# dharunm236/TempME

Measured on AMD Instinct MI355X. Metric: explained target-edges/sec (TGN+Enron, n_degree=20) at 1/2/4/8 MI355X, higher is better.
Workload: dtype fp32

## Files before the change

tempme_amd/csrc/encoder.hip:

```cpp
#include <algorithm>
#include <atomic>
#include <cstring>
#include <vector>

#include "encoder_common.h"

namespace tmk {

__device__ __forceinline__ double block_sum(double v, double *red) {
#pragma unroll
    for (int o = 32; o > 0; o >>= 1) v += __shfl_xor(v, o);
    const int wave = threadIdx.x >> 6, nw = blockDim.x >> 6;
    __syncthreads();
    if ((threadIdx.x & 63) == 0) red[wave] = v;
    __syncthreads();
    double s = 0.0;
    for (int k = 0; k < nw; ++k) s += red[k];
    return s;
}

__global__ void __launch_bounds__(1024) std_kernel(int32_t B, int32_t W, const double *__restrict__ cut,
                                                   const float *__restrict__ ts3, float *__restrict__ std_out) {
    __shared__ double red[16];
    const int64_t g = blockIdx.x;
// ... 525 lines not shown

template <int NQE>
struct WalkLay {
    static constexpr int EV = FoldLay::SIZE, EVB = EV + 11 * NQE * 256, G1 = EVB + 176, G1B = G1 + 4 * 11 * 256,
                         G2 = G1B + 64, G2B = G2 + 4 * 4 * 256, W1 = G2B + 64, W1B = W1 + 8 * 8 * 256, W2 = W1B + 128,
                         W2B = W2 + 8 * 8 * 256, A1 = W2B + 128, A1B = A1 + 4 * 8 * 256, A2 = A1B + 64,
                         A2B = A2 + 4 * 4 * 256, M1 = A2B + 64, M1B = M1 + 5 * 5 * 256, M2 = M1B + 80,
                         M2B = M2 + 4 * 5 * 256;
};

constexpr int PFP = 4;
constexpr int WALK_WAVES = 2;
constexpr int WALK_WPB = 4;

constexpr int GCN_LDS = 3;
constexpr int GCN_LDS_FRAGS = GCN_LDS * 12;
constexpr int PAIR_LIN_RING = 6, PAIR_GCN_RING = 6;
constexpr int gcn_step(int k, int gl, int ns) {
    const int nstr = ns - gl, m = nstr < gl ? nstr : gl;
    if (k < 2 * m) return (k & 1) ? k / 2 : gl + k / 2;
    return nstr > gl ? gl + k - m : k - m;
}

template <int NTO, int NQ, int NQL, int BASE>
__device__ __forceinline__ void cgemm(__amdgpu_buffer_rsrc_t wr, const floatx4 (&x)[NQ], floatx4 (&o)[NTO]) {
    using O = PairOrder<NTO, NQ>;
    const int vo = lane_id() * 16;
    constexpr int N = NTO * NQ, D = PFP < N ? PFP : N;
    auto off = [](int i) { return BASE / 4 + (O::t(i) * NQL + O::q(i)) * 64; };
    float4 buf[D];
#pragma unroll
// ... 283 lines not shown
    const float4 v = erow4[i < n4 ? i : n4 - 1];
    return i < n4 ? v : make_float4(0.f, 0.f, 0.f, 0.f);
}

#define ETAB_N(q0) ((q0) > 0 ? 11 : 1)
template <int Q0>
__device__ __forceinline__ void load_et(const WalkArgs &a, int32_t e, float4 (&et)[ETAB_N(Q0)]) {
    if constexpr (Q0 > 0) {
        const float4 *trow = reinterpret_cast<const float4 *>(a.etab + (int64_t)e * 176);
        const int g = lane_id() >> 4;
#pragma unroll
        for (int t = 0; t < 11; ++t) et[t] = trow[4 * t + g];
    }
}

template <int NTD, bool AGAIN, int D, class Extra>
__device__ __forceinline__ void gcn_zn(__amdgpu_buffer_rsrc_t wr, int vog, const float4 *gl, const floatx4 (&L)[NTD],
                                       float4 (&gb)[D], Extra &&extra, floatx4 (&Hs)[4], float4 (&pre)[PFP],
                                       const NextFr &nx) {
    constexpr int NSG = (NTD + 1) / 2, GL = GCN_LDS, N = (NSG - GL) * 12;
    static_assert(N % D == 0 && D >= PFP, "event_gcn ring depth");
    const int vo = lane_id() * 16, ln = lane_id();
    auto goff = [](int i) { return ((((i / 3) % 4) * NSG + GL + i / 12) * 3 + i % 3) * 64; };
    int zg = 0;
    asm volatile("" : "+s"(zg));
    auto wloadg = [&](int i) {
        return __builtin_bit_cast(float4, __builtin_amdgcn_raw_buffer_load_b128(wr, vog, zg + goff(i) * 16, 0));
    };
    auto take = [&](int i) {
        const float4 v = gb[i % D];
        if (i + D < N) gb[i % D] = wloadg(i + D);
        else if constexpr (AGAIN) gb[i % D] = wloadg(i + D - N);
        else if (i + D - N < PFP) gb[i % D] = wload(wr, vo, nx.o[i + D - N]);
        return v;
    };
    auto fetch = [&](int p, float4 (&w)[6]) {
        const int u = gcn_step(p / 2, GL, NSG), t = 2 * (p & 1);
#pragma unroll
        for (int k = 0; k < 6; ++k) {
            if (u < GL) w[k] = gl[((u * 4 + t) * 3 + k) * 64 + ln];
            else w[k] = take(((u - GL) * 4 + t) * 3 + k);
        }
    };
    auto act = [&](Split3 &x, int u, int j) {
        const int q = 2 * u + (j >> 2);
        if (q < NTD) {
            split_put(x, j, 0.f + relu(0.f + L[q < NTD ? q : 0][j & 3]));
        } else {
            x.h[j] = (__bf16)0.f;
            x.m[j] = (__bf16)0.f;
            x.l[j] = (__bf16)0.f;
        }
    };
    Split3 xb;
#pragma unroll
    for (int j = 0; j < 8; ++j) act(xb, gcn_step(0, GL, NSG), j);
    float4 wb[2][6];
    fetch(0, wb[0]);
#pragma unroll
    for (int k = 0; k < NSG; ++k) {
        extra(2 * k);
        if (2 * k + 1 < NTD) extra(2 * k + 1);
        Split3 xn = xb;
#pragma unroll
        for (int t = 0; t < 4; t += 2) {
            const int pp = 2 * k + t / 2;
            if (pp + 1 < 2 * NSG) fetch(pp + 1, wb[(pp + 1) & 1]);
            const float4(&w)[6] = wb[pp & 1];
            const bf16x8 h0 = __builtin_bit_cast(bf16x8, w[0]), m0 = __builtin_bit_cast(bf16x8, w[1]),
                         l0 = __builtin_bit_cast(bf16x8, w[2]), h1 = __builtin_bit_cast(bf16x8, w[3]),
                         m1 = __builtin_bit_cast(bf16x8, w[4]), l1 = __builtin_bit_cast(bf16x8, w[5]);
            Hs[t] = TM_MF32(l0, xb.h, Hs[t]);
            Hs[t + 1] = TM_MF32(l1, xb.h, Hs[t + 1]);
            Hs[t] = TM_MF32(h0, xb.l, Hs[t]);
            Hs[t + 1] = TM_MF32(h1, xb.l, Hs[t + 1]);
            Hs[t] = TM_MF32(m0, xb.m, Hs[t]);
            Hs[t + 1] = TM_MF32(m1, xb.m, Hs[t + 1]);
            Hs[t] = TM_MF32(m0, xb.h, Hs[t]);
            Hs[t + 1] = TM_MF32(m1, xb.h, Hs[t + 1]);
            Hs[t] = TM_MF32(h0, xb.m, Hs[t]);
            Hs[t + 1] = TM_MF32(h1, xb.m, Hs[t + 1]);
            Hs[t] = TM_MF32(h0, xb.h, Hs[t]);
            Hs[t + 1] = TM_MF32(h1, xb.h, Hs[t + 1]);
            if (k + 1 < NSG) {
#pragma unroll
                for (int j = 2 * t; j < 2 * t + 4; ++j) act(xn, gcn_step(k + 1, GL, NSG), j);
            }
            __builtin_amdgcn_sched_barrier(0);
        }
        xb = xn;
    }
    if constexpr (!AGAIN) {
#pragma unroll
        for (int k = 0; k < PFP; ++k) pre[k] = gb[(N + k) % D];
    }
}

template <int NQE, int NTD, bool SEF, int Q0, bool ZN, class Extra>
__device__ __forceinline__ void encode_position(const WalkArgs &a, __amdgpu_buffer_rsrc_t wr, const float *cs,
                                                const PosIn &pi, const float (&ef)[EQ_MAX][4],
                                                float4 (&et)[ETAB_N(Q0)], Extra &&extra, int p, floatx4 (&H)[8],
                                                float4 (&pre)[PFP], const NextFr &nx, unsigned long long (&T)[10],
                                                const float4 *gl) {
    constexpr bool ETAB = Q0 > 0;
    static_assert(!(ETAB && SEF), "table mode replaces the streamed edge features");
    using C = WalkConsts<NQE, NTD>;
    using LY = WalkLay<NQE>;
    const EncW &P = a.P;
    const int g = lane_id() >> 4;
    const int de = P.de, dn = P.dn;
    const float dt = pi.v ? pi.tb - pi.ta : 0.f, c0 = pi.v ? pi.c0 : 0.f, c1 = pi.v ? pi.c1 : 0.f,
                c2 = pi.v ? pi.c2 : 0.f;
    const float4 *nrow_s = reinterpret_cast<const float4 *>(a.n_feat + (int64_t)(pi.v ? pi.ns : 0) * dn);
    const float4 *nrow_t = reinterpret_cast<const float4 *>(a.n_feat + (int64_t)(pi.v ? pi.nt : 0) * dn);
    floatx4 L[NTD];
    if constexpr (ETAB) {
#pragma unroll
        for (int t = 0; t < NTD; ++t) L[t] = floatx4{et[t].x, et[t].y, et[t].z, et[t].w};
        if (p == 2) {
#pragma unroll
            for (int t = 0; t < NTD; ++t) L[t] = add4(L[t], lds4(cs + C::DEVC, t));
        }
    } else {
        const float *bias = cs + (p == 2 ? C::EVC : C::EV);
#pragma unroll
        for (int t = 0; t < NTD; ++t) L[t] = ldsx4(bias, t);
    }
    TM_STAMP(1);
    constexpr int NSG = (NTD + 1) / 2, GD = 12, GL = GCN_LDS;
    static_assert(GL >= 1 && GL < NSG, "event_gcn's resident steps");
    const int vog = lane_id() * 16 + 16 * (int)(P.g13 - P.kv.w);
    auto goff = [](int i) { return ((((i / 3) % 4) * NSG + GL + i / 12) * 3 + i % 3) * 64; };
    float4 gb[ZN ? GD : 1];
    (void)vog, (void)goff, (void)gb;
    constexpr int JN = 3;
    float4 rs[JN], rt[JN];
    auto nload = [&](int q) {
        const int f4 = (q < NTD - 1) ? 4 * q + g : min(4 * q + g, dn / 4 - 1);
        rs[q % JN] = nrow_s[f4];
        rt[q % JN] = nrow_t[f4];
    };
    {
        constexpr int NS = C::NS, S0 = Q0 / 2;
        constexpr int N = NTD * (NS - S0) * 3, D = 12;
        static_assert(D >= PFP && D <= N && D % 3 == 0, "lin_event ring depth");
        static_assert(D == GD, "the zero-node event_gcn takes over lin_event's ring slots");
        const int vo = lane_id() * 16;
        const int vo3 = vo + 16 * (int)(P.ev3 - P.kv.w);
// ... 47 lines not shown
                        e2[1] = ef_step(erow4, s + 2, 1, g, de);
                    }
                }
                Split3 xn = xs;
                auto gen = [&](int j) {
                    if (s + 1 < NS && j < 8) {
                        const float e = edge(s + 1, j);
                        const float v = pure(s + 1) ? gen_one<ETAB, true>(s + 1, j, w8[j], p8[j], e, g, de, dt, c0, c1, c2)
                                                    : gen_one<ETAB, false>(s + 1, j, w8[j], p8[j], e, g, de, dt, c0, c1, c2);
                        split_put(xn, j, v);
                    }
                };
                auto take = [&](int i) {
                    const bf16x8 v = __builtin_bit_cast(bf16x8, buf[i % D]);
                    if (i + D < N) buf[i % D] = wload3(i + D);
                    else if constexpr (ZN) buf[i % D] = wloadg(i + D - N);
                    else if (i + D - N < PFP) buf[i % D] = wload(wr, vo, g1f(i + D - N));
                    return v;
                };
#pragma unroll
                for (int t = 0; t + 1 < NTD; t += 2) {
                    const int i = ((s - S0) * NTD + t) * 3;
                    const bf16x8 h0 = take(i), m0 = take(i + 1), l0 = take(i + 2);
                    const bf16x8 h1 = take(i + 3), m1 = take(i + 4), l1 = take(i + 5);
                    L[t] = TM_MF32(l0, xs.h, L[t]);
                    L[t + 1] = TM_MF32(l1, xs.h, L[t + 1]);
                    L[t] = TM_MF32(h0, xs.l, L[t]);
                    L[t + 1] = TM_MF32(h1, xs.l, L[t + 1]);
                    L[t] = TM_MF32(m0, xs.m, L[t]);
                    L[t + 1] = TM_MF32(m1, xs.m, L[t + 1]);
                    L[t] = TM_MF32(m0, xs.h, L[t]);
// ... 14 lines not shown
                    L[t] = TM_MF32(h0, xs.l, L[t]);
                    L[t] = TM_MF32(m0, xs.m, L[t]);
                    L[t] = TM_MF32(m0, xs.h, L[t]);
                    L[t] = TM_MF32(h0, xs.m, L[t]);
                    L[t] = TM_MF32(h0, xs.h, L[t]);
                    gen(t);
                    __builtin_amdgcn_sched_barrier(0);
                }
                if constexpr (SEF) {
                    ring[s & 1][0] = e2[0];
                    ring[s & 1][1] = e2[1];
                }
                xs = xn;
            }
        }
        if constexpr (ZN) {
            if (p == 2) {
#pragma unroll
                for (int k = 0; k < D; ++k) buf[(N + k) % D] = wloadg(k);
            }
#pragma unroll
            for (int k = 0; k < D; ++k) gb[k] = buf[(N + k) % D];
        } else {
            if (p == 2) {
#pragma unroll
                for (int k = 0; k < PFP; ++k) buf[(N + k) % D] = wload(wr, vo, g1f(k));
            }
#pragma unroll
            for (int k = 0; k < PFP; ++k) pre[k] = buf[(N + k) % D];
        }
    }
    TM_STAMP(2);
    floatx4 Hs[4], Ht[4];
#pragma unroll
    for (int t = 0; t < 4; ++t) {
        Hs[t] = ldsx4(cs + C::G1, t);
        if constexpr (!ZN) Ht[t] = ldsx4(cs + C::G1C, t);
    }
    if constexpr (ZN) {
        gcn_zn<NTD, false, GD>(wr, vog, gl, L, gb, extra, Hs, pre, nx);
    } else {
        const int vo = lane_id() * 16;
        float4 wq[2][4];
        {
#pragma unroll
            for (int q = 0; q < JN - 1 && q < NTD; ++q) nload(q);
        }
#pragma unroll
        for (int t = 0; t < 4; ++t) wq[0][t] = pre[t];
#pragma unroll
        for (int q = 0; q < NTD; ++q) {
            if (q + JN - 1 < NTD) nload(q + JN - 1);
            if (q + 1 < NTD) {
#pragma unroll
                for (int t = 0; t < 4; ++t) wq[(q + 1) & 1][t] = wload(wr, vo, LY::G1 / 4 + (t * NTD + q + 1) * 64);
// ... 26 lines not shown
            __builtin_amdgcn_sched_barrier(0);
        }
#pragma unroll
        for (int t = 0; t < 4; ++t) pre[t] = wq[NTD & 1][t];
    }
    TM_STAMP(3);
    TM_STAMP(4);
#pragma unroll
    for (int t = 0; t < 4; ++t) {
        H[t] = relu4(Hs[t]);
        H[4 + t] = ZN ? H[t] : relu4(Ht[t]);
    }
    TM_STAMP(5);
}

template <int NQE, int NTD, int Q0, class Extra>
__device__ __forceinline__ void encode_pair(const WalkArgs &a, __amdgpu_buffer_rsrc_t wr, const float *cs,
                                            const PosIn &pi0, const PosIn &pi1, const float4 (&et0)[NTD],
                                            const float4 (&et1)[NTD], Extra &&extra, floatx4 (&U0)[4],
                                            floatx4 (&U1)[4], float4 (&pre)[PFP], const NextFr &nx,
                                            unsigned long long (&T)[10], const float4 *gl) {
    static_assert(Q0 > 0, "the pair pass starts from the edge table's rows");
    using C = WalkConsts<NQE, NTD>;
    const EncW &P = a.P;
    const int g = lane_id() >> 4;
    const int de = P.de;
    const float dt0 = pi0.v ? pi0.tb - pi0.ta : 0.f, c00 = pi0.v ? pi0.c0 : 0.f, c01 = pi0.v ? pi0.c1 : 0.f,
                c02 = pi0.v ? pi0.c2 : 0.f;
    const float dt1 = pi1.v ? pi1.tb - pi1.ta : 0.f, c10 = pi1.v ? pi1.c0 : 0.f, c11 = pi1.v ? pi1.c1 : 0.f,
                c12 = pi1.v ? pi1.c2 : 0.f;
    floatx4 L0[NTD], L1[NTD];
#pragma unroll
    for (int t = 0; t < NTD; ++t) {
        L0[t] = floatx4{et0[t].x, et0[t].y, et0[t].z, et0[t].w};
        L1[t] = floatx4{et1[t].x, et1[t].y, et1[t].z, et1[t].w};
    }
    TM_STAMP(1);
    constexpr int NSG = (NTD + 1) / 2, GL = GCN_LDS;
    const int vog = lane_id() * 16 + 16 * (int)(P.g13 - P.kv.w);
    constexpr int GD = PAIR_GCN_RING;
    float4 gb[GD];
    {
        constexpr int NS = C::NS, S0 = Q0 / 2;
        constexpr int N = NTD * (NS - S0) * 3, D = PAIR_LIN_RING;
        static_assert(D >= PFP && D <= N && D % 3 == 0 && D <= GD, "lin_event ring depth");
        const int vo3 = lane_id() * 16 + 16 * (int)(P.ev3 - P.kv.w);
        auto off = [](int i) { return ((((i / 3) % NTD) * NS + S0 + i / (3 * NTD)) * 3 + i % 3) * 64; };
        auto goff = [](int i) { return ((((i / 3) % 4) * NSG + GL + i / 12) * 3 + i % 3) * 64; };
        int z3 = 0;
        asm volatile("" : "+s"(z3));
        auto wload3 = [&](int i) {
            return __builtin_bit_cast(float4, __builtin_amdgcn_raw_buffer_load_b128(wr, vo3, z3 + off(i) * 16, 0));
        };
        auto wloadg = [&](int i) {
            return __builtin_bit_cast(float4, __builtin_amdgcn_raw_buffer_load_b128(wr, vog, z3 + goff(i) * 16, 0));
        };
        float4 buf[D];
#pragma unroll
        for (int i = 0; i < D; ++i) buf[i] = i < PFP ? pre[i] : wload3(i);
        auto pure = [](int s) { return s > S0; };
        const float *cw = cs + C::XW, *cp = cs + C::XP;
        Split3 xs0, xs1;
        {
            float w8[8], p8[8];
            lds8(cw, S0, w8);
            lds8(cp, S0, p8);
#pragma unroll
            for (int j = 0; j < 8; ++j) {
                split_put(xs0, j, gen_one<true, false>(S0, j, w8[j], p8[j], 0.f, g, de, dt0, c00, c01, c02));
                split_put(xs1, j, gen_one<true, false>(S0, j, w8[j], p8[j], 0.f, g, de, dt1, c10, c11, c12));
            }
// ... 3 lines not shown
            Split3 xn0 = xs0, xn1 = xs1;
            auto gen = [&](int j) {
                if (s + 1 < NS && j < 8) {
                    const float w = cw[32 * (s + 1) + 8 * g + j], ph = cp[32 * (s + 1) + 8 * g + j];
                    const float v0 = pure(s + 1) ? gen_one<true, true>(s + 1, j, w, ph, 0.f, g, de, dt0, c00, c01, c02)
                                                 : gen_one<true, false>(s + 1, j, w, ph, 0.f, g, de, dt0, c00, c01, c02);
                    const float v1 = pure(s + 1) ? gen_one<true, true>(s + 1, j, w, ph, 0.f, g, de, dt1, c10, c11, c12)
                                                 : gen_one<true, false>(s + 1, j, w, ph, 0.f, g, de, dt1, c10, c11, c12);
                    split_put(xn0, j, v0);
                    split_put(xn1, j, v1);
                }
            };
            auto take = [&](int i) {
                const bf16x8 v = __builtin_bit_cast(bf16x8, buf[i % D]);
                if (i + D < N) buf[i % D] = wload3(i + D);
                else buf[i % D] = wloadg(i + D - N);
                return v;
            };
#pragma unroll
            for (int t = 0; t < NTD; ++t) {
                const int i = ((s - S0) * NTD + t) * 3;
                const bf16x8 h = take(i), m = take(i + 1), l = take(i + 2);
                L0[t] = TM_MF32(l, xs0.h, L0[t]);
                L1[t] = TM_MF32(l, xs1.h, L1[t]);
                L0[t] = TM_MF32(h, xs0.l, L0[t]);
                L1[t] = TM_MF32(h, xs1.l, L1[t]);
                L0[t] = TM_MF32(m, xs0.m, L0[t]);
                L1[t] = TM_MF32(m, xs1.m, L1[t]);
                L0[t] = TM_MF32(m, xs0.h, L0[t]);
                L1[t] = TM_MF32(m, xs1.h, L1[t]);
                L0[t] = TM_MF32(h, xs0.m, L0[t]);
                L1[t] = TM_MF32(h, xs1.m, L1[t]);
                L0[t] = TM_MF32(h, xs0.h, L0[t]);
                L1[t] = TM_MF32(h, xs1.h, L1[t]);
                gen(t);
                __builtin_amdgcn_sched_barrier(0);
            }
            xs0 = xn0;
            xs1 = xn1;
        }
#pragma unroll
        for (int k = 0; k < GD; ++k) gb[k] = k < D ? buf[(N + k) % D] : wloadg(k);
    }
    TM_STAMP(2);
    floatx4 Hs[4];
#pragma unroll
    for (int t = 0; t < 4; ++t) Hs[t] = ldsx4(cs + C::G1, t);
    gcn_zn<NTD, true, GD>(wr, vog, gl, L0, gb, [](int) {}, Hs, pre, nx);
#pragma unroll
    for (int t = 0; t < 4; ++t) U0[t] = relu4(Hs[t]);
    TM_STAMP(3);
#pragma unroll
    for (int t = 0; t < 4; ++t) Hs[t] = ldsx4(cs + C::G1, t);
    gcn_zn<NTD, false, GD>(wr, vog, gl, L1, gb, extra, Hs, pre, nx);
    TM_STAMP(4);
#pragma unroll
    for (int t = 0; t < 4; ++t) U1[t] = relu4(Hs[t]);
    TM_STAMP(5);
}

__device__ __forceinline__ float col_sum(float v) {
    v += __shfl_xor(v, 16);
    v += __shfl_xor(v, 32);
    return v;
}

struct HeadIn {
    double cu;
    float sd, t0, t1;
// ... 105 lines not shown
__device__ __forceinline__ float score_dot(const Stash<ZN ? 4 : 8> &st, const floatx4 (&H)[NH]) {
    static_assert(NH >= (ZN ? 4 : 8), "a position's hidden vector");
    const int lane = threadIdx.x & 63;
    float s = 0.f;
#pragma unroll
    for (int t = 0; t < (ZN ? 4 : 8); ++t) {
        const floatx4 v = st.V[t][lane];
#pragma unroll
        for (int r = 0; r < 4; ++r) s = __builtin_fmaf(v[r], H[t][r], s);
    }
    return col_sum(s) + st.cw[lane];
}

template <int NQE, int NTD, bool SEF = false, int QE0 = 0, bool SPLIT = false, bool ZN = false, bool POOL = false,
          bool PAIR = false>
__global__ void __launch_bounds__(64 * WALK_WPB, 4 * WALK_WAVES / WALK_WPB) walk_kernel(WalkArgs a) {
    static_assert(!PAIR || (ZN && QE0 > 0 && !SEF && !POOL), "the pair pass: zero-node table mode, not pooled");
    using C = WalkConsts<NQE, NTD>;
    constexpr int NA = ZN ? 4 : 8;
    const EncW &P = a.P;
    const int lane = threadIdx.x & 63, col = lane & 15;
    const int32_t NS = a.W / a.M;
    const int64_t n_units = (a.n_slots + 15) / 16;
    constexpr bool PERSIST = !SPLIT;
    const int64_t ustride = PERSIST ? (int64_t)gridDim.x * (blockDim.x >> 6) : n_units;
    int64_t unit = (int64_t)blockIdx.x * (blockDim.x >> 6) + (threadIdx.x >> 6);
    auto ticket = [&]() -> int64_t {
        uint32_t t = 0;
        if (lane == 0) t = atomicAdd(a.ticket, 1u);
        return ustride + (int64_t)(uint32_t)__builtin_amdgcn_readfirstlane((int)t);
    };
    int m0 = 0;
    if constexpr (SPLIT) {
        m0 = (int)(unit % a.M);
        unit /= a.M;
    }
    auto coords = [&](int64_t u, bool &v, int64_t &eg_, int32_t &j_) {
        const int64_t gs = u * 16 + col;
        v = u < n_units && gs < a.n_slots;
        eg_ = v ? gs / NS : 0;
        j_ = v ? (int32_t)(gs % NS) : 0;
    };
    bool valid;
    int64_t eg;
    int32_t j;
    coords(unit, valid, eg, j);
    __shared__ Stash<NA> stash[WALK_WPB];
    __shared__ float4 cs4[(C::SIZE + 3) / 4];
    float *cs = reinterpret_cast<float *>(cs4);
#ifdef TM_TRACE
    const int64_t trw = (int64_t)blockIdx.x * (blockDim.x >> 6) + (threadIdx.x >> 6);
    int trn = 0;
    const unsigned long long tr0 = __builtin_amdgcn_s_memrealtime();
#endif
    __shared__ float4 gl[ZN ? GCN_LDS_FRAGS * 64 : 1];
    if constexpr (ZN) {
        constexpr int NSG = (NTD + 1) / 2;
        for (int i = threadIdx.x; i < GCN_LDS_FRAGS * 64; i += blockDim.x) {
            const int f = i >> 6, l = i & 63;
            gl[i] = P.g13[((((f / 3) % 4) * NSG + f / 12) * 3 + f % 3) * 64 + l];
        }
    }
    load_consts<NQE, NTD, ZN>(P, cs);
    __syncthreads();
#ifdef TM_TRACE
    if (lane == 0 && trw < 8192) {
        g_tr[trw][0] = tr0;
        g_tr[trw][1] = __builtin_amdgcn_s_memrealtime();
        g_tr[trw][28] = 0;
        g_tr[trw][29] = (unsigned)__builtin_amdgcn_s_getreg(63492) | ((unsigned long long)(unsigned)__builtin_amdgcn_s_getreg(30740) << 32);
    }
#endif
    if (unit >= n_units) return;
// ... 61 lines not shown
        const int64_t gwn = !last ? eg * a.W + (int64_t)j * a.M + (SPLIT ? m0 : PAIR ? pass : pass >> 1)
                                  : egn * a.W + (int64_t)jn * a.M;
        PosIn nxt, nxt1;
        auto extra = [&](int q) {
            if (q == 0) {
                load_hi();
                nxt = load_pos(a, gwn, pn, !last ? valid : vn);
                if constexpr (PAIR) nxt1 = load_pos(a, gwn, 1, !last ? valid : vn);
            }
        };
        unsigned long long T[10];
        TM_STAMP(0);
        if (PAIR && pt == 3) {
            if constexpr (PAIR) {
                floatx4 U0[4], U1[4];
                encode_pair<NQE, NTD, QE0>(a, wr, cs, cur, cur1, et, et1, extra, U0, U1, pre,
                                           pair_first<4>(FoldLay::A1GZ / 4), T, gl);
                load_et<QE0>(a, nxt.edge(), et);
                load_et<QE0>(a, nxt1.edge(), et1);
                cur = nxt;
                cur1 = nxt1;
                TM_STAMP(6);
                const float sc0 = score_dot<true>(st, U0), sc1 = score_dot<true>(st, U1);
                TM_STAMP(7);
                walk_head<NQE, NTD, true>(a, wr, cs, gw, valid, hi, st, sc0, sc1, U0, U1, pre, lin0);
            }
        } else {
        const int p = PAIR ? 2 : pt;
        floatx4 H[8];
        const NextFr nx_pos = ZN ? pair_first<4>(p == 2 ? FoldLay::A1DZ / 4 : FoldLay::A1GZ / 4)
                                 : pair_first<8>(p == 2 ? FoldLay::A1D / 4 : FoldLay::A1G / 4);
        encode_position<NQE, NTD, SEF, QE0, ZN>(a, wr, cs, cur, ef, et, extra, p, H, pre,
                                                p == 0 ? lin0 : nx_pos, T, gl);
        if constexpr (QE0 == 0) load_ef(a, nxt.edge(), ef);
        else load_et<QE0>(a, nxt.edge(), et);
        cur = nxt;
        if constexpr (PAIR) {
            load_et<QE0>(a, nxt1.edge(), et1);
            cur1 = nxt1;
        }
        TM_STAMP(6);
        floatx4 Uv[4];
#pragma unroll
        for (int t = 0; t < 4; ++t) Uv[t] = H[t];
        if (ZN && p == 2) {
            floatx4 P2[4], V[4];
#pragma unroll
// ... 663 lines not shown
                        const uint8_t *drop, float dscale, hipStream_t s) {
    const int tr = head_tr(P);
    if (tr == 32)
        head_kernel<32><<<dim3((unsigned)((n_walks + 31) / 32)), 256, head_lds(P, 32), s>>>(
            P, n_walks, walks_per_group, W, F, ts3, cut, cat, stdv, out, drop, dscale);
    else
        head_kernel<16><<<dim3((unsigned)((n_walks + 15) / 16)), 256, head_lds(P, 16), s>>>(
            P, n_walks, walks_per_group, W, F, ts3, cut, cat, stdv, out, drop, dscale);
}

constexpr int64_t WALK_SPLIT_UNITS = 512;

static bool walk_split(int64_t units, int32_t M) { return units * M <= 3 * WALK_SPLIT_UNITS && units < WALK_SPLIT_UNITS; }

template <int NQE, bool SEF, int Q0, bool ZN, bool POOL, bool PAIR>
static void launch_walk_as(const WalkArgs &a, unsigned blocks, hipStream_t s) {
    const int64_t units = (a.n_slots + 15) / 16;
    if (walk_split(units, a.M)) {
        const unsigned sb = (unsigned)((units * a.M + WALK_WPB - 1) / WALK_WPB);
        walk_kernel<NQE, 11, SEF, Q0, true, ZN, POOL, PAIR><<<dim3(sb), 64 * WALK_WPB, 0, s>>>(a);
        return;
    }
    static int cap[64] = {};
    int dev = 0;
    if (hipGetDevice(&dev) == hipSuccess && dev >= 0 && dev < 64) {
        if (cap[dev] == 0) {
            int per_cu = 0, cus = 0;
            if (hipOccupancyMaxActiveBlocksPerMultiprocessor(&per_cu, walk_kernel<NQE, 11, SEF, Q0, false, ZN, POOL, PAIR>, 64 * WALK_WPB, 0) ==
                    hipSuccess &&
                hipDeviceGetAttribute(&cus, hipDeviceAttributeMultiprocessorCount, dev) == hipSuccess && per_cu > 0 &&
                cus > 0)
                cap[dev] = per_cu * cus;
            else
                cap[dev] = -1;
        }
        if (cap[dev] > 0 && blocks > (unsigned)cap[dev]) blocks = (unsigned)cap[dev];
    }
    const int dbg = debug_opt(TM_DEBUG_WALK_BLOCKS);
    if (dbg > 0 && blocks > (unsigned)dbg) blocks = (unsigned)dbg;
    walk_kernel<NQE, 11, SEF, Q0, false, ZN, POOL, PAIR><<<dim3(blocks), 64 * WALK_WPB, 0, s>>>(a);
}

template <int NQE, bool SEF = false, int Q0 = 0, bool ZN = false, bool POOL = false>
static void launch_walk(const WalkArgs &a, unsigned blocks, hipStream_t s) {
    if constexpr (ZN && Q0 > 0 && !SEF && !POOL) {
        if (!debug_opt(TM_DEBUG_WALK_SINGLE)) return launch_walk_as<NQE, SEF, Q0, ZN, POOL, true>(a, blocks, s);
    }
    launch_walk_as<NQE, SEF, Q0, ZN, POOL, false>(a, blocks, s);
}

extern "C" int tm_encoder_fwd(const tm_weights *w, const float *n_feat, const float *e_feat, int32_t n_groups,
                              int32_t B, int32_t W, int32_t M, const int32_t *node6, const int32_t *eid3,
                              const float *ts3, const int32_t *cat, const double *cut, const float *cnt,
                              void *workspace, float *out_imp, void *stream) {
    return tm_encoder_fwd_tab(w, n_feat, e_feat, nullptr, n_groups, B, W, M, node6, eid3, ts3, cat, cut, cnt,
                              workspace, out_imp, stream);
}

static int encoder_fwd_impl(const tm_weights *w, const float *n_feat, const float *e_feat, const float *etab,
                            int32_t n_groups, int32_t B, int32_t W, int32_t M, const int32_t *node6, const int32_t *eid3,
                            const float *ts3, const int32_t *cat, const double *cut, const float *cnt, void *workspace,
                            float *out_imp, void *stream, bool do_std);

// ... 26 lines not shown
        pe = prof_begin(s);
        if (P.tg) std_kernel<<<dim3(n_groups), 1024, 0, s>>>(B, W, cut, ts3, stdv);
        TM_CHECK_LAUNCH();
        prof_end("std_kernel", s, pe);
    }
    if (etab && etab_q0(P) == 0) return fail(TM_E_UNSUPPORTED, "tm_encoder_fwd_tab: no edge table for these dims");
    const int nqe = r16(P.kev) / 16, ntd = r16(P.dn) / 16;
    const bool narrow = nqe >= 11 && nqe <= 14 && P.de <= 16 * EQ_MAX;
    const bool wide = (nqe == 21 || nqe == 22) && P.de > 16 * EQ_MAX && P.de % 4 == 0;
    if (ntd == 11 && P.dn % 4 == 0 && (narrow || wide) && P.h == HID && P.cat) {
        if (!walk_layout_ok(P, nqe)) return fail(TM_E_UNSUPPORTED, "tm_encoder_fwd: weight layout mismatch");
        const int64_t n_slots = n_walks / M;
        const int64_t units = (n_slots + 15) / 16;
        WalkArgs a{P, n_slots, W, M, B * W, n_feat, e_feat, node6, eid3, cat, ts3, cnt, stdv, cut, out_imp, etab,
                   reinterpret_cast<uint32_t *>(F)};
        const unsigned blocks = (unsigned)((units + WALK_WPB - 1) / WALK_WPB);
        const int q0 = etab ? etab_q0(P) : 0;
        if (!walk_split(units, M)) TM_HIP(hipMemsetAsync(a.ticket, 0, sizeof(uint32_t), s));
        pe = prof_begin(s);
        if (q0 == 2 && w->node_zero) {
            if (nqe == 11) launch_walk<11, false, 2, true>(a, blocks, s);
            else if (nqe == 12) launch_walk<12, false, 2, true>(a, blocks, s);
            else if (nqe == 13) launch_walk<13, false, 2, true>(a, blocks, s);
            else launch_walk<14, false, 2, true>(a, blocks, s);
        } else if (q0 == 2) {
            if (nqe == 11) launch_walk<11, false, 2>(a, blocks, s);
            else if (nqe == 12) launch_walk<12, false, 2>(a, blocks, s);
            else if (nqe == 13) launch_walk<13, false, 2>(a, blocks, s);
            else launch_walk<14, false, 2>(a, blocks, s);
        } else if (q0 == 10) {
            if (nqe == 21) launch_walk<21, false, 10>(a, blocks, s);
            else launch_walk<22, false, 10>(a, blocks, s);
        } else if (wide) {
            if (nqe == 21) launch_walk<21, true>(a, blocks, s);
            else launch_walk<22, true>(a, blocks, s);
        } else if (nqe == 11) launch_walk<11>(a, blocks, s);
        else if (nqe == 12) launch_walk<12>(a, blocks, s);
        else if (nqe == 13) launch_walk<13>(a, blocks, s);
        else launch_walk<14>(a, blocks, s);
        TM_CHECK_LAUNCH();
        prof_end("walk_kernel", s, pe);
        return TM_OK;
    }
    const int64_t n_rows = n_walks * 3;
    pe = prof_begin(s);
    launch_gcn(P, w->node_zero, n_rows, lds_g, n_feat, e_feat, node6, eid3, ts3, cnt, F, s);
    TM_CHECK_LAUNCH();
    prof_end("gcn_kernel", s, pe);
    pe = prof_begin(s);
    launch_head(P, n_walks, (int64_t)B * W, W, F, ts3, cut, cat, stdv, out_imp, nullptr, 1.f, s);
    TM_CHECK_LAUNCH();
    prof_end("head_kernel", s, pe);
    return TM_OK;
}

static int64_t pool_part_offset(const tm_weights *w, int64_t n_walks) {
    return (tm_encoder_workspace_bytes(w, n_walks) + 255) & ~(int64_t)255;
}

extern "C" int64_t tm_encoder_pool_workspace_bytes(const tm_weights *w, int64_t n_walks) {
    return pool_part_offset(w, n_walks) + n_walks * (w ? w->h : HID) * (int64_t)sizeof(float) + 256;
}

static void launch_walk_pool(const WalkArgs &a, int nqe, bool wide, int q0, int node_zero, unsigned blocks,
                             hipStream_t s) {
    if (q0 == 2 && node_zero) {
        if (nqe == 11) launch_walk<11, false, 2, true, true>(a, blocks, s);
        else if (nqe == 12) launch_walk<12, false, 2, true, true>(a, blocks, s);
        else if (nqe == 13) launch_walk<13, false, 2, true, true>(a, blocks, s);
        else launch_walk<14, false, 2, true, true>(a, blocks, s);
    } else if (q0 == 2) {
        if (nqe == 11) launch_walk<11, false, 2, false, true>(a, blocks, s);
        else if (nqe == 12) launch_walk<12, false, 2, false, true>(a, blocks, s);
        else if (nqe == 13) launch_walk<13, false, 2, false, true>(a, blocks, s);
        else launch_walk<14, false, 2, false, true>(a, blocks, s);
    } else if (q0 == 10) {
        if (nqe == 21) launch_walk<21, false, 10, false, true>(a, blocks, s);
        else launch_walk<22, false, 10, false, true>(a, blocks, s);
    } else if (wide) {
        if (nqe == 21) launch_walk<21, true, 0, false, true>(a, blocks, s);
        else launch_walk<22, true, 0, false, true>(a, blocks, s);
    } else if (nqe == 11) launch_walk<11, false, 0, false, true>(a, blocks, s);
    else if (nqe == 12) launch_walk<12, false, 0, false, true>(a, blocks, s);
    else if (nqe == 13) launch_walk<13, false, 0, false, true>(a, blocks, s);
    else launch_walk<14, false, 0, false, true>(a, blocks, s);
}

extern "C" int tm_encoder_pool_fwd(const tm_weights *w, const float *n_feat, const float *e_feat, const float *etab,
                                   int32_t n_groups, int32_t B, int32_t W, int32_t M, const int32_t *node6,
                                   const int32_t *eid3, const float *ts3, const int32_t *cat, const double *cut,
                                   const float *cnt, const float *wgt, void *workspace, float *out, int64_t ld_out,
                                   void *stream) {
    if (!w || n_groups < 0 || B < 0 || W < 0 || M <= 0) return fail(TM_E_ARG, "tm_encoder_pool_fwd: bad arguments");
    if (W % M) return fail(TM_E_SHAPE, "tm_encoder_pool_fwd: W must be a multiple of M (walks per hop-1 slot)");
    const int64_t n_walks = (int64_t)n_groups * B * W, n_events = (int64_t)n_groups * B;
    if (n_events == 0) return TM_OK;
    const EncW &P = w->P;
    if (ld_out < P.hm) return fail(TM_E_ARG, "tm_encoder_pool_fwd: ld_out below the row width (hid_dim (+ 12))");
    if (!n_feat || !e_feat || !node6 || !eid3 || !ts3 || !cat || !cut || !cnt || !wgt || !workspace || !out)
        return fail(TM_E_ARG, "tm_encoder_pool_fwd: NULL pointer");
// ... 7 lines not shown
    if (n_walks > 0) {
        hipEvent_t pe = prof_begin(s);
        if (P.tg) std_kernel<<<dim3(n_groups), 1024, 0, s>>>(B, W, cut, ts3, stdv);
        TM_CHECK_LAUNCH();
        prof_end("std_kernel", s, pe);
        if (etab && etab_q0(P) == 0) return fail(TM_E_UNSUPPORTED, "tm_encoder_pool_fwd: no edge table for these dims");
        const int nqe = r16(P.kev) / 16, ntd = r16(P.dn) / 16;
        const bool narrow = nqe >= 11 && nqe <= 14 && P.de <= 16 * EQ_MAX;
        const bool wide = (nqe == 21 || nqe == 22) && P.de > 16 * EQ_MAX && P.de % 4 == 0;
        if (ntd == 11 && P.dn % 4 == 0 && (narrow || wide) && P.h == HID && P.cat) {
            if (!walk_layout_ok(P, nqe)) return fail(TM_E_UNSUPPORTED, "tm_encoder_pool_fwd: weight layout mismatch");
            const int64_t n_slots = n_walks / M;
            const int64_t units = (n_slots + 15) / 16;
            WalkArgs a{P, n_slots, W, M, B * W, n_feat, e_feat, node6, eid3, cat, ts3, cnt, stdv, cut, part, etab,
                       reinterpret_cast<uint32_t *>(F), wgt};
            const unsigned blocks = (unsigned)((units + WALK_WPB - 1) / WALK_WPB);
            const bool split = walk_split(units, M);
            if (!split) TM_HIP(hipMemsetAsync(a.ticket, 0, sizeof(uint32_t), s));
            n_part = split ? W : W / M;
            pe = prof_begin(s);
            launch_walk_pool(a, nqe, wide, etab ? etab_q0(P) : 0, w->node_zero, blocks, s);
            TM_CHECK_LAUNCH();
            prof_end("walk_pool_kernel", s, pe);
        } else {
            pe = prof_begin(s);
            launch_gcn(P, w->node_zero, n_walks * 3, lds_g, n_feat, e_feat, node6, eid3, ts3, cnt, F, s);
            TM_CHECK_LAUNCH();
            prof_end("gcn_kernel", s, pe);
            pe = prof_begin(s);
            head_kernel<16, true><<<dim3((unsigned)((n_walks + 15) / 16)), 256, head_lds(P, 16), s>>>(
                P, n_walks, (int64_t)B * W, W, F, ts3, cut, cat, stdv, part, nullptr, 1.f, wgt);
            TM_CHECK_LAUNCH();
            prof_end("head_pool_kernel", s, pe);
        }
    }
    hipEvent_t pe = prof_begin(s);
// ... 493 lines not shown
```

Before: 3.725 million.

## Keep all GCN weight steps resident in LDS with 8-wave workgroups

For zero-node, non-split walk kernels (pair or pooled), the workgroup grows from 4 to 8 waves and the whole GCN weight tile for all steps is staged in LDS, so gcn_zn no longer streams weight fragments through a register ring from global memory. The ring buffers and their prefetch logic are compiled out in resident mode, and the next-stage prefetch is issued directly instead. This aims to cut repeated global weight loads and free ring registers, at the cost of more LDS per block and changed launch bounds, which may lower occupancy. Launchers now compute the block count from the per-variant waves-per-block.

After: 3.955 million, median of 6. 1.06x the previous value.

```diff
diff --git a/tempme_amd/csrc/encoder.hip b/tempme_amd/csrc/encoder.hip
--- a/tempme_amd/csrc/encoder.hip
+++ b/tempme_amd/csrc/encoder.hip
@@ -563,7 +563,14 @@
 constexpr int WALK_WPB = 4;
 
 constexpr int GCN_LDS = 3;
-constexpr int GCN_LDS_FRAGS = GCN_LDS * 12;
+#ifndef TM_WALK_WG8
+#define TM_WALK_WG8 1
+#endif
+constexpr bool walk_wg8(bool zn, bool pair, bool split, bool pool) { return TM_WALK_WG8 && zn && !split && (pair || pool); }
+constexpr int walk_wpb(bool zn, bool pair, bool split, bool pool) { return walk_wg8(zn, pair, split, pool) ? 8 : WALK_WPB; }
+constexpr int walk_gl(bool zn, bool pair, bool split, bool pool, int nsg) {
+    return walk_wg8(zn, pair, split, pool) ? nsg : GCN_LDS;
+}
 constexpr int PAIR_LIN_RING = 6, PAIR_GCN_RING = 6;
 constexpr int gcn_step(int k, int gl, int ns) {
     const int nstr = ns - gl, m = nstr < gl ? nstr : gl;
@@ -877,12 +884,14 @@
     }
 }
 
-template <int NTD, bool AGAIN, int D, class Extra>
+template <int NTD, bool AGAIN, int GL, int D, class Extra>
 __device__ __forceinline__ void gcn_zn(__amdgpu_buffer_rsrc_t wr, int vog, const float4 *gl, const floatx4 (&L)[NTD],
                                        float4 (&gb)[D], Extra &&extra, floatx4 (&Hs)[4], float4 (&pre)[PFP],
                                        const NextFr &nx) {
-    constexpr int NSG = (NTD + 1) / 2, GL = GCN_LDS, N = (NSG - GL) * 12;
-    static_assert(N % D == 0 && D >= PFP, "event_gcn ring depth");
+    constexpr int NSG = (NTD + 1) / 2, N = (NSG - GL) * 12;
+    constexpr bool RES = GL == NSG;
+    static_assert(GL >= 1 && GL <= NSG, "event_gcn's resident steps");
+    static_assert(RES || (N % D == 0 && D >= PFP), "event_gcn ring depth");
     const int vo = lane_id() * 16, ln = lane_id();
     auto goff = [](int i) { return ((((i / 3) % 4) * NSG + GL + i / 12) * 3 + i % 3) * 64; };
     int zg = 0;
@@ -898,10 +907,10 @@
         return v;
     };
     auto fetch = [&](int p, float4 (&w)[6]) {
-        const int u = gcn_step(p / 2, GL, NSG), t = 2 * (p & 1);
+        const int u = gcn_step(p / 2, GCN_LDS, NSG), t = 2 * (p & 1);
 #pragma unroll
         for (int k = 0; k < 6; ++k) {
-            if (u < GL) w[k] = gl[((u * 4 + t) * 3 + k) * 64 + ln];
+            if (RES || u < GL) w[k] = gl[((u * 4 + t) * 3 + k) * 64 + ln];
             else w[k] = take(((u - GL) * 4 + t) * 3 + k);
         }
     };
@@ -917,7 +926,7 @@
     };
     Split3 xb;
 #pragma unroll
-    for (int j = 0; j < 8; ++j) act(xb, gcn_step(0, GL, NSG), j);
+    for (int j = 0; j < 8; ++j) act(xb, gcn_step(0, GCN_LDS, NSG), j);
     float4 wb[2][6];
     fetch(0, wb[0]);
 #pragma unroll
@@ -947,19 +956,19 @@
             Hs[t + 1] = TM_MF32(h1, xb.h, Hs[t + 1]);
             if (k + 1 < NSG) {
 #pragma unroll
-                for (int j = 2 * t; j < 2 * t + 4; ++j) act(xn, gcn_step(k + 1, GL, NSG), j);
+                for (int j = 2 * t; j < 2 * t + 4; ++j) act(xn, gcn_step(k + 1, GCN_LDS, NSG), j);
             }
             __builtin_amdgcn_sched_barrier(0);
         }
         xb = xn;
     }
-    if constexpr (!AGAIN) {
+    if constexpr (!AGAIN && !RES) {
 #pragma unroll
         for (int k = 0; k < PFP; ++k) pre[k] = gb[(N + k) % D];
     }
 }
 
-template <int NQE, int NTD, bool SEF, int Q0, bool ZN, class Extra>
+template <int NQE, int NTD, bool SEF, int Q0, bool ZN, int GL, class Extra>
 __device__ __forceinline__ void encode_position(const WalkArgs &a, __amdgpu_buffer_rsrc_t wr, const float *cs,
                                                 const PosIn &pi, const float (&ef)[EQ_MAX][4],
                                                 float4 (&et)[ETAB_N(Q0)], Extra &&extra, int p, floatx4 (&H)[8],
@@ -990,11 +999,12 @@
         for (int t = 0; t < NTD; ++t) L[t] = ldsx4(bias, t);
     }
     TM_STAMP(1);
-    constexpr int NSG = (NTD + 1) / 2, GD = 12, GL = GCN_LDS;
-    static_assert(GL >= 1 && GL < NSG, "event_gcn's resident steps");
+    constexpr int NSG = (NTD + 1) / 2, GD = 12;
+    constexpr bool RES = ZN && GL == NSG;
+    static_assert(!ZN || (GL >= 1 && GL <= NSG), "event_gcn's resident steps");
     const int vog = lane_id() * 16 + 16 * (int)(P.g13 - P.kv.w);
     auto goff = [](int i) { return ((((i / 3) % 4) * NSG + GL + i / 12) * 3 + i % 3) * 64; };
-    float4 gb[ZN ? GD : 1];
+    float4 gb[ZN && !RES ? GD : 1];
     (void)vog, (void)goff, (void)gb;
     constexpr int JN = 3;
     float4 rs[JN], rt[JN];
@@ -1072,7 +1082,9 @@
                 auto take = [&](int i) {
                     const bf16x8 v = __builtin_bit_cast(bf16x8, buf[i % D]);
                     if (i + D < N) buf[i % D] = wload3(i + D);
-                    else if constexpr (ZN) buf[i % D] = wloadg(i + D - N);
+                    else if constexpr (RES) {
+                        if (i + D - N < PFP) buf[i % D] = wload(wr, vo, nx.o[i + D - N]);
+                    } else if constexpr (ZN) buf[i % D] = wloadg(i + D - N);
                     else if (i + D - N < PFP) buf[i % D] = wload(wr, vo, g1f(i + D - N));
                     return v;
                 };
@@ -1117,7 +1129,14 @@
                 xs = xn;
             }
         }
-        if constexpr (ZN) {
+        if constexpr (RES) {
+            if (p == 2) {
+#pragma unroll
+                for (int k = 0; k < PFP; ++k) buf[(N + k) % D] = wload(wr, vo, nx.o[k]);
+            }
+#pragma unroll
+            for (int k = 0; k < PFP; ++k) pre[k] = buf[(N + k) % D];
+        } else if constexpr (ZN) {
             if (p == 2) {
 #pragma unroll
                 for (int k = 0; k < D; ++k) buf[(N + k) % D] = wloadg(k);
@@ -1141,7 +1160,7 @@
         if constexpr (!ZN) Ht[t] = ldsx4(cs + C::G1C, t);
     }
     if constexpr (ZN) {
-        gcn_zn<NTD, false, GD>(wr, vog, gl, L, gb, extra, Hs, pre, nx);
+        gcn_zn<NTD, false, GL, RES ? 1 : GD>(wr, vog, gl, L, gb, extra, Hs, pre, nx);
     } else {
         const int vo = lane_id() * 16;
         float4 wq[2][4];
@@ -1198,7 +1217,7 @@
     TM_STAMP(5);
 }
 
-template <int NQE, int NTD, int Q0, class Extra>
+template <int NQE, int NTD, int Q0, int GL, class Extra>
 __device__ __forceinline__ void encode_pair(const WalkArgs &a, __amdgpu_buffer_rsrc_t wr, const float *cs,
                                             const PosIn &pi0, const PosIn &pi1, const float4 (&et0)[NTD],
                                             const float4 (&et1)[NTD], Extra &&extra, floatx4 (&U0)[4],
@@ -1220,14 +1239,17 @@
         L1[t] = floatx4{et1[t].x, et1[t].y, et1[t].z, et1[t].w};
     }
     TM_STAMP(1);
-    constexpr int NSG = (NTD + 1) / 2, GL = GCN_LDS;
+    constexpr int NSG = (NTD + 1) / 2;
+    constexpr bool RES = GL == NSG;
     const int vog = lane_id() * 16 + 16 * (int)(P.g13 - P.kv.w);
-    constexpr int GD = PAIR_GCN_RING;
+    constexpr int GD = RES ? 1 : PAIR_GCN_RING;
     float4 gb[GD];
+    (void)vog, (void)gb;
     {
         constexpr int NS = C::NS, S0 = Q0 / 2;
         constexpr int N = NTD * (NS - S0) * 3, D = PAIR_LIN_RING;
-        static_assert(D >= PFP && D <= N && D % 3 == 0 && D <= GD, "lin_event ring depth");
+        static_assert(D >= PFP && D <= N && D % 3 == 0 && (RES || D <= GD), "lin_event ring depth");
+        const int vo = lane_id() * 16;
         const int vo3 = lane_id() * 16 + 16 * (int)(P.ev3 - P.kv.w);
         auto off = [](int i) { return ((((i / 3) % NTD) * NS + S0 + i / (3 * NTD)) * 3 + i % 3) * 64; };
         auto goff = [](int i) { return ((((i / 3) % 4) * NSG + GL + i / 12) * 3 + i % 3) * 64; };
@@ -1239,6 +1261,7 @@
         auto wloadg = [&](int i) {
             return __builtin_bit_cast(float4, __builtin_amdgcn_raw_buffer_load_b128(wr, vog, z3 + goff(i) * 16, 0));
         };
+        (void)wloadg, (void)vo;
         float4 buf[D];
 #pragma unroll
         for (int i = 0; i < D; ++i) buf[i] = i < PFP ? pre[i] : wload3(i);
@@ -1272,7 +1295,9 @@
             auto take = [&](int i) {
                 const bf16x8 v = __builtin_bit_cast(bf16x8, buf[i % D]);
                 if (i + D < N) buf[i % D] = wload3(i + D);
-                else buf[i % D] = wloadg(i + D - N);
+                else if constexpr (RES) {
+                    if (i + D - N < PFP) buf[i % D] = wload(wr, vo, nx.o[i + D - N]);
+                } else buf[i % D] = wloadg(i + D - N);
                 return v;
             };
 #pragma unroll
@@ -1297,20 +1322,25 @@
             xs0 = xn0;
             xs1 = xn1;
         }
-#pragma unroll
-        for (int k = 0; k < GD; ++k) gb[k] = k < D ? buf[(N + k) % D] : wloadg(k);
+        if constexpr (RES) {
+#pragma unroll
+            for (int k = 0; k < PFP; ++k) pre[k] = buf[(N + k) % D];
+        } else {
+#pragma unroll
+            for (int k = 0; k < GD; ++k) gb[k] = k < D ? buf[(N + k) % D] : wloadg(k);
+        }
     }
     TM_STAMP(2);
     floatx4 Hs[4];
 #pragma unroll
     for (int t = 0; t < 4; ++t) Hs[t] = ldsx4(cs + C::G1, t);
-    gcn_zn<NTD, true, GD>(wr, vog, gl, L0, gb, [](int) {}, Hs, pre, nx);
+    gcn_zn<NTD, true, GL, GD>(wr, vog, gl, L0, gb, [](int) {}, Hs, pre, nx);
 #pragma unroll
     for (int t = 0; t < 4; ++t) U0[t] = relu4(Hs[t]);
     TM_STAMP(3);
 #pragma unroll
     for (int t = 0; t < 4; ++t) Hs[t] = ldsx4(cs + C::G1, t);
-    gcn_zn<NTD, false, GD>(wr, vog, gl, L1, gb, extra, Hs, pre, nx);
+    gcn_zn<NTD, false, GL, GD>(wr, vog, gl, L1, gb, extra, Hs, pre, nx);
     TM_STAMP(4);
 #pragma unroll
     for (int t = 0; t < 4; ++t) U1[t] = relu4(Hs[t]);
@@ -1446,9 +1476,11 @@
 
 template <int NQE, int NTD, bool SEF = false, int QE0 = 0, bool SPLIT = false, bool ZN = false, bool POOL = false,
           bool PAIR = false>
-__global__ void __launch_bounds__(64 * WALK_WPB, 4 * WALK_WAVES / WALK_WPB) walk_kernel(WalkArgs a) {
+__global__ void __launch_bounds__(64 * walk_wpb(ZN, PAIR, SPLIT, POOL), WALK_WAVES) walk_kernel(WalkArgs a) {
     static_assert(!PAIR || (ZN && QE0 > 0 && !SEF && !POOL), "the pair pass: zero-node table mode, not pooled");
     using C = WalkConsts<NQE, NTD>;
+    constexpr int WPB = walk_wpb(ZN, PAIR, SPLIT, POOL);
+    constexpr int GL = walk_gl(ZN, PAIR, SPLIT, POOL, (NTD + 1) / 2);
     constexpr int NA = ZN ? 4 : 8;
     const EncW &P = a.P;
     const int lane = threadIdx.x & 63, col = lane & 15;
@@ -1477,7 +1509,7 @@
     int64_t eg;
     int32_t j;
     coords(unit, valid, eg, j);
-    __shared__ Stash<NA> stash[WALK_WPB];
+    __shared__ Stash<NA> stash[WPB];
     __shared__ float4 cs4[(C::SIZE + 3) / 4];
     float *cs = reinterpret_cast<float *>(cs4);
 #ifdef TM_TRACE
@@ -1485,10 +1517,10 @@
     int trn = 0;
     const unsigned long long tr0 = __builtin_amdgcn_s_memrealtime();
 #endif
-    __shared__ float4 gl[ZN ? GCN_LDS_FRAGS * 64 : 1];
+    __shared__ float4 gl[ZN ? GL * 12 * 64 : 1];
     if constexpr (ZN) {
         constexpr int NSG = (NTD + 1) / 2;
-        for (int i = threadIdx.x; i < GCN_LDS_FRAGS * 64; i += blockDim.x) {
+        for (int i = threadIdx.x; i < GL * 12 * 64; i += blockDim.x) {
             const int f = i >> 6, l = i & 63;
             gl[i] = P.g13[((((f / 3) % 4) * NSG + f / 12) * 3 + f % 3) * 64 + l];
         }
@@ -1580,7 +1612,7 @@
         if (PAIR && pt == 3) {
             if constexpr (PAIR) {
                 floatx4 U0[4], U1[4];
-                encode_pair<NQE, NTD, QE0>(a, wr, cs, cur, cur1, et, et1, extra, U0, U1, pre,
+                encode_pair<NQE, NTD, QE0, GL>(a, wr, cs, cur, cur1, et, et1, extra, U0, U1, pre,
                                            pair_first<4>(FoldLay::A1GZ / 4), T, gl);
                 load_et<QE0>(a, nxt.edge(), et);
                 load_et<QE0>(a, nxt1.edge(), et1);
@@ -1596,7 +1628,7 @@
         floatx4 H[8];
         const NextFr nx_pos = ZN ? pair_first<4>(p == 2 ? FoldLay::A1DZ / 4 : FoldLay::A1GZ / 4)
                                  : pair_first<8>(p == 2 ? FoldLay::A1D / 4 : FoldLay::A1G / 4);
-        encode_position<NQE, NTD, SEF, QE0, ZN>(a, wr, cs, cur, ef, et, extra, p, H, pre,
+        encode_position<NQE, NTD, SEF, QE0, ZN, GL>(a, wr, cs, cur, ef, et, extra, p, H, pre,
                                                 p == 0 ? lin0 : nx_pos, T, gl);
         if constexpr (QE0 == 0) load_ef(a, nxt.edge(), ef);
         else load_et<QE0>(a, nxt.edge(), et);
@@ -2290,19 +2322,22 @@
 static bool walk_split(int64_t units, int32_t M) { return units * M <= 3 * WALK_SPLIT_UNITS && units < WALK_SPLIT_UNITS; }
 
 template <int NQE, bool SEF, int Q0, bool ZN, bool POOL, bool PAIR>
-static void launch_walk_as(const WalkArgs &a, unsigned blocks, hipStream_t s) {
+static void launch_walk_as(const WalkArgs &a, hipStream_t s) {
     const int64_t units = (a.n_slots + 15) / 16;
     if (walk_split(units, a.M)) {
-        const unsigned sb = (unsigned)((units * a.M + WALK_WPB - 1) / WALK_WPB);
-        walk_kernel<NQE, 11, SEF, Q0, true, ZN, POOL, PAIR><<<dim3(sb), 64 * WALK_WPB, 0, s>>>(a);
+        constexpr int WPB = walk_wpb(ZN, PAIR, true, POOL);
+        const unsigned sb = (unsigned)((units * a.M + WPB - 1) / WPB);
+        walk_kernel<NQE, 11, SEF, Q0, true, ZN, POOL, PAIR><<<dim3(sb), 64 * WPB, 0, s>>>(a);
         return;
     }
+    constexpr int WPB = walk_wpb(ZN, PAIR, false, POOL);
+    unsigned blocks = (unsigned)((units + WPB - 1) / WPB);
     static int cap[64] = {};
     int dev = 0;
     if (hipGetDevice(&dev) == hipSuccess && dev >= 0 && dev < 64) {
         if (cap[dev] == 0) {
             int per_cu = 0, cus = 0;
-            if (hipOccupancyMaxActiveBlocksPerMultiprocessor(&per_cu, walk_kernel<NQE, 11, SEF, Q0, false, ZN, POOL, PAIR>, 64 * WALK_WPB, 0) ==
+            if (hipOccupancyMaxActiveBlocksPerMultiprocessor(&per_cu, walk_kernel<NQE, 11, SEF, Q0, false, ZN, POOL, PAIR>, 64 * WPB, 0) ==
                     hipSuccess &&
                 hipDeviceGetAttribute(&cus, hipDeviceAttributeMultiprocessorCount, dev) == hipSuccess && per_cu > 0 &&
                 cus > 0)
@@ -2314,15 +2349,15 @@
     }
     const int dbg = debug_opt(TM_DEBUG_WALK_BLOCKS);
     if (dbg > 0 && blocks > (unsigned)dbg) blocks = (unsigned)dbg;
-    walk_kernel<NQE, 11, SEF, Q0, false, ZN, POOL, PAIR><<<dim3(blocks), 64 * WALK_WPB, 0, s>>>(a);
+    walk_kernel<NQE, 11, SEF, Q0, false, ZN, POOL, PAIR><<<dim3(blocks), 64 * WPB, 0, s>>>(a);
 }
 
 template <int NQE, bool SEF = false, int Q0 = 0, bool ZN = false, bool POOL = false>
-static void launch_walk(const WalkArgs &a, unsigned blocks, hipStream_t s) {
+static void launch_walk(const WalkArgs &a, hipStream_t s) {
     if constexpr (ZN && Q0 > 0 && !SEF && !POOL) {
-        if (!debug_opt(TM_DEBUG_WALK_SINGLE)) return launch_walk_as<NQE, SEF, Q0, ZN, POOL, true>(a, blocks, s);
-    }
-    launch_walk_as<NQE, SEF, Q0, ZN, POOL, false>(a, blocks, s);
+        if (!debug_opt(TM_DEBUG_WALK_SINGLE)) return launch_walk_as<NQE, SEF, Q0, ZN, POOL, true>(a, s);
+    }
+    launch_walk_as<NQE, SEF, Q0, ZN, POOL, false>(a, s);
 }
 
 extern "C" int tm_encoder_fwd(const tm_weights *w, const float *n_feat, const float *e_feat, int32_t n_groups,
@@ -2379,30 +2414,29 @@
         const int64_t units = (n_slots + 15) / 16;
         WalkArgs a{P, n_slots, W, M, B * W, n_feat, e_feat, node6, eid3, cat, ts3, cnt, stdv, cut, out_imp, etab,
                    reinterpret_cast<uint32_t *>(F)};
-        const unsigned blocks = (unsigned)((units + WALK_WPB - 1) / WALK_WPB);
         const int q0 = etab ? etab_q0(P) : 0;
         if (!walk_split(units, M)) TM_HIP(hipMemsetAsync(a.ticket, 0, sizeof(uint32_t), s));
         pe = prof_begin(s);
         if (q0 == 2 && w->node_zero) {
-            if (nqe == 11) launch_walk<11, false, 2, true>(a, blocks, s);
-            else if (nqe == 12) launch_walk<12, false, 2, true>(a, blocks, s);
-            else if (nqe == 13) launch_walk<13, false, 2, true>(a, blocks, s);
-            else launch_walk<14, false, 2, true>(a, blocks, s);
+            if (nqe == 11) launch_walk<11, false, 2, true>(a, s);
+            else if (nqe == 12) launch_walk<12, false, 2, true>(a, s);
+            else if (nqe == 13) launch_walk<13, false, 2, true>(a, s);
+            else launch_walk<14, false, 2, true>(a, s);
         } else if (q0 == 2) {
-            if (nqe == 11) launch_walk<11, false, 2>(a, blocks, s);
-            else if (nqe == 12) launch_walk<12, false, 2>(a, blocks, s);
-            else if (nqe == 13) launch_walk<13, false, 2>(a, blocks, s);
-            else launch_walk<14, false, 2>(a, blocks, s);
+            if (nqe == 11) launch_walk<11, false, 2>(a, s);
+            else if (nqe == 12) launch_walk<12, false, 2>(a, s);
+            else if (nqe == 13) launch_walk<13, false, 2>(a, s);
+            else launch_walk<14, false, 2>(a, s);
         } else if (q0 == 10) {
-            if (nqe == 21) launch_walk<21, false, 10>(a, blocks, s);
-            else launch_walk<22, false, 10>(a, blocks, s);
+            if (nqe == 21) launch_walk<21, false, 10>(a, s);
+            else launch_walk<22, false, 10>(a, s);
         } else if (wide) {
-            if (nqe == 21) launch_walk<21, true>(a, blocks, s);
-            else launch_walk<22, true>(a, blocks, s);
-        } else if (nqe == 11) launch_walk<11>(a, blocks, s);
-        else if (nqe == 12) launch_walk<12>(a, blocks, s);
-        else if (nqe == 13) launch_walk<13>(a, blocks, s);
-        else launch_walk<14>(a, blocks, s);
+            if (nqe == 21) launch_walk<21, true>(a, s);
+            else launch_walk<22, true>(a, s);
+        } else if (nqe == 11) launch_walk<11>(a, s);
+        else if (nqe == 12) launch_walk<12>(a, s);
+        else if (nqe == 13) launch_walk<13>(a, s);
+        else launch_walk<14>(a, s);
         TM_CHECK_LAUNCH();
         prof_end("walk_kernel", s, pe);
         return TM_OK;
@@ -2427,28 +2461,27 @@
     return pool_part_offset(w, n_walks) + n_walks * (w ? w->h : HID) * (int64_t)sizeof(float) + 256;
 }
 
-static void launch_walk_pool(const WalkArgs &a, int nqe, bool wide, int q0, int node_zero, unsigned blocks,
-                             hipStream_t s) {
+static void launch_walk_pool(const WalkArgs &a, int nqe, bool wide, int q0, int node_zero, hipStream_t s) {
     if (q0 == 2 && node_zero) {
-        if (nqe == 11) launch_walk<11, false, 2, true, true>(a, blocks, s);
-        else if (nqe == 12) launch_walk<12, false, 2, true, true>(a, blocks, s);
-        else if (nqe == 13) launch_walk<13, false, 2, true, true>(a, blocks, s);
-        else launch_walk<14, false, 2, true, true>(a, blocks, s);
+        if (nqe == 11) launch_walk<11, false, 2, true, true>(a, s);
+        else if (nqe == 12) launch_walk<12, false, 2, true, true>(a, s);
+        else if (nqe == 13) launch_walk<13, false, 2, true, true>(a, s);
+        else launch_walk<14, false, 2, true, true>(a, s);
     } else if (q0 == 2) {
-        if (nqe == 11) launch_walk<11, false, 2, false, true>(a, blocks, s);
-        else if (nqe == 12) launch_walk<12, false, 2, false, true>(a, blocks, s);
-        else if (nqe == 13) launch_walk<13, false, 2, false, true>(a, blocks, s);
-        else launch_walk<14, false, 2, false, true>(a, blocks, s);
+        if (nqe == 11) launch_walk<11, false, 2, false, true>(a, s);
+        else if (nqe == 12) launch_walk<12, false, 2, false, true>(a, s);
+        else if (nqe == 13) launch_walk<13, false, 2, false, true>(a, s);
+        else launch_walk<14, false, 2, false, true>(a, s);
     } else if (q0 == 10) {
-        if (nqe == 21) launch_walk<21, false, 10, false, true>(a, blocks, s);
-        else launch_walk<22, false, 10, false, true>(a, blocks, s);
+        if (nqe == 21) launch_walk<21, false, 10, false, true>(a, s);
+        else launch_walk<22, false, 10, false, true>(a, s);
     } else if (wide) {
-        if (nqe == 21) launch_walk<21, true, 0, false, true>(a, blocks, s);
-        else launch_walk<22, true, 0, false, true>(a, blocks, s);
-    } else if (nqe == 11) launch_walk<11, false, 0, false, true>(a, blocks, s);
-    else if (nqe == 12) launch_walk<12, false, 0, false, true>(a, blocks, s);
-    else if (nqe == 13) launch_walk<13, false, 0, false, true>(a, blocks, s);
-    else launch_walk<14, false, 0, false, true>(a, blocks, s);
+        if (nqe == 21) launch_walk<21, true, 0, false, true>(a, s);
+        else launch_walk<22, true, 0, false, true>(a, s);
+    } else if (nqe == 11) launch_walk<11, false, 0, false, true>(a, s);
+    else if (nqe == 12) launch_walk<12, false, 0, false, true>(a, s);
+    else if (nqe == 13) launch_walk<13, false, 0, false, true>(a, s);
+    else launch_walk<14, false, 0, false, true>(a, s);
 }
 
 extern "C" int tm_encoder_pool_fwd(const tm_weights *w, const float *n_feat, const float *e_feat, const float *etab,
@@ -2486,12 +2519,11 @@
             const int64_t units = (n_slots + 15) / 16;
             WalkArgs a{P, n_slots, W, M, B * W, n_feat, e_feat, node6, eid3, cat, ts3, cnt, stdv, cut, part, etab,
                        reinterpret_cast<uint32_t *>(F), wgt};
-            const unsigned blocks = (unsigned)((units + WALK_WPB - 1) / WALK_WPB);
             const bool split = walk_split(units, M);
             if (!split) TM_HIP(hipMemsetAsync(a.ticket, 0, sizeof(uint32_t), s));
             n_part = split ? W : W / M;
             pe = prof_begin(s);
-            launch_walk_pool(a, nqe, wide, etab ? etab_q0(P) : 0, w->node_zero, blocks, s);
+            launch_walk_pool(a, nqe, wide, etab ? etab_q0(P) : 0, w->node_zero, s);
             TM_CHECK_LAUNCH();
             prof_end("walk_pool_kernel", s, pe);
         } else {
```
